# Arsham-001/tsu-emulator

Hardware: AMD Instinct MI355X
Metric: spin-updates/sec on L×L 2D Ising Gibbs sweep; achieved HBM GB/s vs peak (higher is better)
Workload: dtype int8

## Files before the change

### tsu-emulator_amd/csrc/ising2d_tiled.hip

```cpp
#include "ising2d.h"

#include <type_traits>
#include <vector>

typedef short v2s __attribute__((ext_vector_type(2)));
typedef unsigned short v2us __attribute__((ext_vector_type(2)));

struct TiledParams {
    const int8_t* src;
    int8_t* dst;
    long long pitch;
    int rows, nchunks;
    int cols;
    int q_shift;
    int tile_h;
    int flex_ty;
    int r_begin, r_end;
    long long row0, total_rows;
    int wrap_rows, ghost;
    int k;
    int tiles_x;
    int ty_first, ty_stride;
    uint32_t k0, k1, sweep0, tag_hi, tag_lo;
    uint32_t tblH0, tblH1, tblL0, tblL1;
// ... 38 lines not shown

struct PhiloxKeys {
    uint32_t a[10], b[10];
};

static __device__ __forceinline__ PhiloxKeys make_keys(uint32_t k0, uint32_t k1) {
    PhiloxKeys K;
#pragma unroll
    for (int r = 0; r < 10; ++r) {
        uint32_t x = k0 + (uint32_t)r * TSU_PHILOX_W0, y = k1 + (uint32_t)r * TSU_PHILOX_W1;
        asm volatile("v_mov_b32 %0, %1" : "=v"(x) : "s"(x));
        asm volatile("v_mov_b32 %0, %1" : "=v"(y) : "s"(y));
        K.a[r] = x;
        K.b[r] = y;
    }
    return K;
}

static __device__ __forceinline__ u32x4 philox_vk(uint32_t c0, uint32_t c1, uint32_t c2, uint32_t c3, const PhiloxKeys& K) {
#pragma unroll
    for (int r = 0; r < 10; ++r) {
        uint64_t p0 = (uint64_t)TSU_PHILOX_M0 * c0;
        uint64_t p1 = (uint64_t)TSU_PHILOX_M1 * c2;
        uint32_t n0 = tsu_xor3((uint32_t)(p1 >> 32), c1, K.a[r]);
        uint32_t n2 = tsu_xor3((uint32_t)(p0 >> 32), c3, K.b[r]);
        c1 = (uint32_t)p1;
        c3 = (uint32_t)p0;
        c0 = n0;
        c2 = n2;
    }
    return u32x4{c0, c1, c2, c3};
}

struct Rows2Ctx {
    const void* Ps;
    void* Pd;
    const uint64_t* s_thr;
    int tr_lo, npairs;
    int rgf;
    int total_rows;
    int rg_tile0, wrap_tr;
    uint32_t hs, tag_hi, tag_lo, k0, k1;
    uint32_t tblH0, tblH1, tblL0, tblL1;
    uint32_t t3H0, t3H1, t3L0, t3L1;
    int last_row;
    bool lft, rgt;
    uint32_t r_par, r_slot;
    uint32_t rm_lo, rm_hi;
    uint64_t vm_e, vm_o;
    int sh_next, sh_prev;
};

static __device__ __forceinline__ u32x4 compare_octet(const u32x4& w, uint32_t cnt_lo, uint32_t cnt_hi, uint32_t tH0,
                                                      uint32_t tH1, uint32_t tL0, uint32_t tL1) {
    const uint32_t Hl = perm(tH1, tH0, cnt_lo), Ll = perm(tL1, tL0, cnt_lo);
    const uint32_t Hh = perm(tH1, tH0, cnt_hi), Lh = perm(tL1, tL0, cnt_hi);
    u32x4 d;
    d.x = subsat16(w.x, perm(Hl, Ll, 0x05010400u));
    d.y = subsat16(w.y, perm(Hl, Ll, 0x07030602u));
    d.z = subsat16(w.z, perm(Hh, Lh, 0x05010400u));
    d.w = subsat16(w.w, perm(Hh, Lh, 0x07030602u));
    return d;
}

static __device__ __forceinline__ u32x4 compare_octet_open(const u32x4& w, uint32_t cnt_lo, uint32_t cnt_hi, const Rows2Ctx& c,
                                                           bool row_edge, bool l0, bool r7) {
    uint32_t Hl = perm(c.tblH1, c.tblH0, cnt_lo), Ll = perm(c.tblL1, c.tblL0, cnt_lo);
    uint32_t Hh = perm(c.tblH1, c.tblH0, cnt_hi), Lh = perm(c.tblL1, c.tblL0, cnt_hi);
    if (row_edge | l0 | r7) {
        const uint32_t rl = r7 ? c.rm_lo : 0u, rh = r7 ? c.rm_hi : 0u;
        const uint32_t il = cnt_lo + ((row_edge && l0) ? 0x00000004u : 0u) + (row_edge ? (rl & 0x04040404u) : 0u);
        const uint32_t ih = cnt_hi + (row_edge ? (rh & 0x04040404u) : 0u);
        const uint32_t ml = row_edge ? 0xFFFFFFFFu : ((l0 ? 0x000000FFu : 0u) | rl), mh = row_edge ? 0xFFFFFFFFu : rh;
        Hl = (Hl & ~ml) | (perm(c.t3H1, c.t3H0, il) & ml);
        Ll = (Ll & ~ml) | (perm(c.t3L1, c.t3L0, il) & ml);
        Hh = (Hh & ~mh) | (perm(c.t3H1, c.t3H0, ih) & mh);
        Lh = (Lh & ~mh) | (perm(c.t3L1, c.t3L0, ih) & mh);
    }
    u32x4 d;
    d.x = subsat16(w.x, perm(Hl, Ll, 0x05010400u));
    d.y = subsat16(w.y, perm(Hl, Ll, 0x07030602u));
    d.z = subsat16(w.z, perm(Hh, Lh, 0x05010400u));
    d.w = subsat16(w.w, perm(Hh, Lh, 0x07030602u));
    return d;
}

static __device__ __forceinline__ bool has_zero_field(const u32x4& d) {
    const uint32_t mn = minu16(minu16(d.x, d.y), minu16(d.z, d.w));
    return ((mn & 0xFFFFu) == 0) | ((mn >> 16) == 0);
}

static __device__ __forceinline__ uint64_t pack_flags(const u32x4& d) {
    const uint32_t nlo = perm(d.y, d.x, 0x0B0A0908u) & 0x01010101u;
    const uint32_t nhi = perm(d.w, d.z, 0x0B0A0908u) & 0x01010101u;
    return (uint64_t)nlo | ((uint64_t)nhi << 32);
}

template <int NO>
static __device__ __forceinline__ void edge_rows(const Rows2Ctx& c, int to_wrap, int tr, int& rga, int& rgb) {
    constexpr int SPAN = 2 * ((NO - 1 + 63) / NO) + 1;
    const int s_off = to_wrap > 0 ? c.rg_tile0 : c.rg_tile0 - c.total_rows;
    rga = tr + s_off;
    rgb = rga + 1;
    if (__builtin_expect((uint32_t)(to_wrap - 1) < (uint32_t)SPAN, 0)) {
        rga = tr + c.rg_tile0;
        asm volatile("" : "+v"(rga));
        rgb = rga + 1;
        if (rga >= c.total_rows) rga -= c.total_rows;
        if (rgb >= c.total_rows) rgb -= c.total_rows;
    }
}

template <int NO, int P0, bool EDGE, bool OPEN, bool SEAM = false>
static __device__ __forceinline__ void sweep_pairs(const Rows2Ctx& c, const PhiloxKeys& K, int tr_first, int tr_end, int step_rows, int oct,
                                                   uint32_t cq) {
    const char* const ps0 = reinterpret_cast<const char*>(c.Ps);
    const int d_off = (int)(reinterpret_cast<const char*>(c.Pd) - ps0);
    const int off_end = tr_end * NO * 8;
    const int off_step = step_rows * NO * 8;
    int off = (tr_first * NO + oct) * 8;
    int rg = EDGE ? tr_first : c.rgf + (tr_first - c.tr_lo);
    int to_wrap = EDGE ? c.wrap_tr - __builtin_amdgcn_readfirstlane(rg) : 0;
#pragma unroll 1
    for (; off < off_end; off += off_step, rg += step_rows, to_wrap -= step_rows) {
        asm volatile("" : "+v"(off), "+v"(rg));
        const char* ps = ps0 + off;
        const uint64_t R0 = *reinterpret_cast<const uint64_t*>(ps - NO * 8), R1 = *reinterpret_cast<const uint64_t*>(ps);
        const uint64_t R2 = *reinterpret_cast<const uint64_t*>(ps + NO * 8), R3 = *reinterpret_cast<const uint64_t*>(ps + 2 * NO * 8);
        const uint32_t A0 = SEAM ? 0u : *reinterpret_cast<const uint32_t*>(ps + (P0 ? 8 : -4));
        const uint32_t A1 = SEAM ? 0u : *reinterpret_cast<const uint32_t*>(ps + NO * 8 + (P0 ? -4 : 8));
        const uint64_t Na = SEAM ? *reinterpret_cast<const uint64_t*>(ps + (P0 ? 8 : -8)) : 0ull;
        const uint64_t Nb = SEAM ? *reinterpret_cast<const uint64_t*>(ps + NO * 8 + (P0 ? -8 : 8)) : 0ull;
        __builtin_amdgcn_sched_barrier(0);
        int rga = rg, rgb = rg + 1;
        if (EDGE) edge_rows<NO>(c, to_wrap, rg, rga, rgb);
        const u32x4 w0 = philox_vk(cq, (uint32_t)rga, c.hs, c.tag_hi, K);
        const u32x4 w1 = philox_vk(cq, (uint32_t)rgb, c.hs, c.tag_hi, K);
        __builtin_amdgcn_sched_barrier(0);
        const uint32_t C0l = (uint32_t)R1, C0h = (uint32_t)(R1 >> 32), C1l = (uint32_t)R2, C1h = (uint32_t)(R2 >> 32);
        uint32_t S0l = P0 ? __builtin_amdgcn_alignbyte(C0h, C0l, 1) : __builtin_amdgcn_alignbyte(C0l, A0, 3);
        uint32_t S0h = P0 ? __builtin_amdgcn_alignbyte(A0, C0h, 1) : __builtin_amdgcn_alignbyte(C0h, C0l, 3);
        uint32_t S1l = P0 ? __builtin_amdgcn_alignbyte(C1l, A1, 3) : __builtin_amdgcn_alignbyte(C1h, C1l, 1);
        uint32_t S1h = P0 ? __builtin_amdgcn_alignbyte(C1h, C1l, 3) : __builtin_amdgcn_alignbyte(A1, C1h, 1);
        if (SEAM) {
            const uint64_t nxa = (Na & 0xFFull) << c.sh_next, pva = (Na >> c.sh_prev) & 0xFFull;
            const uint64_t nxb = (Nb & 0xFFull) << c.sh_next, pvb = (Nb >> c.sh_prev) & 0xFFull;
            const uint64_t Sa = P0 ? ((R1 >> 8) | nxa) : ((R1 << 8) | pva);
            const uint64_t Sb = P0 ? ((R2 << 8) | pvb) : ((R2 >> 8) | nxb);
            S0l = (uint32_t)Sa; S0h = (uint32_t)(Sa >> 32);
            S1l = (uint32_t)Sb; S1h = (uint32_t)(Sb >> 32);
        }
        const uint32_t ml = C0l + C1l, mh = C0h + C1h;
        const uint32_t cnt0l = (uint32_t)R0 + ml + S0l, cnt0h = (uint32_t)(R0 >> 32) + mh + S0h;
        const uint32_t cnt1l = (uint32_t)R3 + ml + S1l, cnt1h = (uint32_t)(R3 >> 32) + mh + S1h;
        u32x4 d0, d1;
        uint32_t edge_a = 0, edge_b = 0;
        if (OPEN) {
            const bool ea = rga == 0 || rga == c.last_row, eb = rgb == 0 || rgb == c.last_row;
            const bool la = !P0 && c.lft, ra = c.rgt && c.r_par == (uint32_t)P0, lb = P0 && c.lft, rb = c.rgt && c.r_par != (uint32_t)P0;
            d0 = compare_octet_open(w0, cnt0l, cnt0h, c, ea, la, ra);
            d1 = compare_octet_open(w1, cnt1l, cnt1h, c, eb, lb, rb);
            edge_a = (ea ? 1u : 0u) | (la ? 2u : 0u) | (ra ? 4u : 0u) | (c.r_slot << 4);
            edge_b = (eb ? 1u : 0u) | (lb ? 2u : 0u) | (rb ? 4u : 0u) | (c.r_slot << 4);
        } else {
            d0 = compare_octet(w0, cnt0l, cnt0h, c.tblH0, c.tblH1, c.tblL0, c.tblL1);
            d1 = compare_octet(w1, cnt1l, cnt1h, c.tblH0, c.tblH1, c.tblL0, c.tblL1);
        }
        const uint32_t mn = minu16(minu16(minu16(d0.x, d0.y), minu16(d0.z, d0.w)), minu16(minu16(d1.x, d1.y), minu16(d1.z, d1.w)));
        if (__builtin_expect(((mn & 0xFFFFu) == 0) | ((mn >> 16) == 0), 0)) {
            if (has_zero_field(d0)) d0 = resolve_ties(d0, w0, cnt0l, cnt0h, c.s_thr, cq, (uint32_t)rga, c.hs, c.tag_lo, c.k0, c.k1, edge_a);
            if (has_zero_field(d1)) d1 = resolve_ties(d1, w1, cnt1l, cnt1h, c.s_thr, cq, (uint32_t)rgb, c.hs, c.tag_lo, c.k0, c.k1, edge_b);
        }
        char* pd = const_cast<char*>(ps) + d_off;
        uint64_t n0 = pack_flags(d0), n1 = pack_flags(d1);
        if (OPEN) {
            n0 = (rga < 0 || rga > c.last_row) ? 0 : (n0 & (P0 ? c.vm_o : c.vm_e));
            n1 = (rgb < 0 || rgb > c.last_row) ? 0 : (n1 & (P0 ? c.vm_e : c.vm_o));
        }
        if (SEAM) {
            n0 &= c.vm_e;
            n1 &= c.vm_e;
        }
        *reinterpret_cast<uint64_t*>(pd) = n0;
        *reinterpret_cast<uint64_t*>(pd + NO * 8) = n1;
    }
}


static __device__ __forceinline__ uint32_t nib_shift_next(uint32_t X, uint32_t N) {
    const uint32_t hi = (N << 4) | __builtin_amdgcn_ubfe(X, 4u, 4u);
    return __builtin_amdgcn_alignbit(hi, X, 8);
}
static __device__ __forceinline__ uint32_t nib_shift_prev(uint32_t X, uint32_t M) {
    const uint32_t w = ((X << 4) & 0x10000000u) | (M >> 4);
    return __builtin_amdgcn_alignbit(X, w, 24);
}
static __device__ __forceinline__ uint32_t nib_shift_next_seam(uint32_t X, uint32_t N, int pos) {
    return nib_shift_next(X, 0u) | ((N & 0xFu) << pos);
}
static __device__ __forceinline__ uint32_t nib_shift_prev_seam(uint32_t X, uint32_t M, int pos) {
    const uint32_t w = ((X << 4) & 0x10000000u) | (((M >> pos) & 0xFu) << 24);
    return __builtin_amdgcn_alignbit(X, w, 24);
}
static __device__ __forceinline__ uint32_t nib_pack(const u32x4& d) {
    const uint64_t f = pack_flags(d);
    return (uint32_t)f | ((uint32_t)(f >> 32) << 4);
}

template <int NO, int P0, bool EDGE, bool OPEN = false, bool SEAM = false>
static __device__ __forceinline__ void sweep_pairs_nib(const Rows2Ctx& c, const PhiloxKeys& K, int tr_first, int tr_end, int step_rows, int oct,
                                                       uint32_t cq) {
    const char* const ps0 = reinterpret_cast<const char*>(c.Ps);
    const int d_off = (int)(reinterpret_cast<const char*>(c.Pd) - ps0);
    const int off_end = tr_end * NO * 4;
    const int off_step = step_rows * NO * 4;
    int off = (tr_first * NO + oct) * 4;
    int rg = EDGE ? tr_first : c.rgf + (tr_first - c.tr_lo);
    int to_wrap = EDGE ? c.wrap_tr - __builtin_amdgcn_readfirstlane(rg) : 0;
#pragma unroll 1
    for (; off < off_end; off += off_step, rg += step_rows, to_wrap -= step_rows) {
        asm volatile("" : "+v"(off), "+v"(rg));
        const char* ps = ps0 + off;
        const uint32_t R0 = *reinterpret_cast<const uint32_t*>(ps - NO * 4), R1 = *reinterpret_cast<const uint32_t*>(ps);
        const uint32_t R2 = *reinterpret_cast<const uint32_t*>(ps + NO * 4), R3 = *reinterpret_cast<const uint32_t*>(ps + 2 * NO * 4);
        const uint32_t A0 = *reinterpret_cast<const uint32_t*>(ps + (P0 ? 4 : -4));
        const uint32_t A1 = *reinterpret_cast<const uint32_t*>(ps + NO * 4 + (P0 ? -4 : 4));
        __builtin_amdgcn_sched_barrier(0);
        int rga = rg, rgb = rg + 1;
        if (EDGE) edge_rows<NO>(c, to_wrap, rg, rga, rgb);
        const u32x4 w0 = philox_vk(cq, (uint32_t)rga, c.hs, c.tag_hi, K);
        const u32x4 w1 = philox_vk(cq, (uint32_t)rgb, c.hs, c.tag_hi, K);
        __builtin_amdgcn_sched_barrier(0);
        const uint32_t Sa = SEAM ? (P0 ? nib_shift_next_seam(R1, A0, c.sh_next) : nib_shift_prev_seam(R1, A0, c.sh_prev))
                                 : (P0 ? nib_shift_next(R1, A0) : nib_shift_prev(R1, A0));
        const uint32_t Sb = SEAM ? (P0 ? nib_shift_prev_seam(R2, A1, c.sh_prev) : nib_shift_next_seam(R2, A1, c.sh_next))
                                 : (P0 ? nib_shift_prev(R2, A1) : nib_shift_next(R2, A1));
        const uint32_t mid = R1 + R2;
        const uint32_t cnt0 = R0 + mid + Sa, cnt1 = R3 + mid + Sb;
        const uint32_t cnt0l = cnt0 & 0x0F0F0F0Fu, cnt0h = (cnt0 >> 4) & 0x0F0F0F0Fu;
        const uint32_t cnt1l = cnt1 & 0x0F0F0F0Fu, cnt1h = (cnt1 >> 4) & 0x0F0F0F0Fu;
        u32x4 d0, d1;
        uint32_t edge_a = 0, edge_b = 0;
        if (OPEN) {
            const bool ea = rga == 0 || rga == c.last_row, eb = rgb == 0 || rgb == c.last_row;
            const bool la = !P0 && c.lft, ra = c.rgt && c.r_par == (uint32_t)P0, lb = P0 && c.lft, rb = c.rgt && c.r_par != (uint32_t)P0;
            d0 = compare_octet_open(w0, cnt0l, cnt0h, c, ea, la, ra);
            d1 = compare_octet_open(w1, cnt1l, cnt1h, c, eb, lb, rb);
            edge_a = (ea ? 1u : 0u) | (la ? 2u : 0u) | (ra ? 4u : 0u) | (c.r_slot << 4);
            edge_b = (eb ? 1u : 0u) | (lb ? 2u : 0u) | (rb ? 4u : 0u) | (c.r_slot << 4);
        } else {
            d0 = compare_octet(w0, cnt0l, cnt0h, c.tblH0, c.tblH1, c.tblL0, c.tblL1);
            d1 = compare_octet(w1, cnt1l, cnt1h, c.tblH0, c.tblH1, c.tblL0, c.tblL1);
        }
        const uint32_t mn = minu16(minu16(minu16(d0.x, d0.y), minu16(d0.z, d0.w)), minu16(minu16(d1.x, d1.y), minu16(d1.z, d1.w)));
        if (__builtin_expect(((mn & 0xFFFFu) == 0) | ((mn >> 16) == 0), 0)) {
            if (has_zero_field(d0)) d0 = resolve_ties(d0, w0, cnt0l, cnt0h, c.s_thr, cq, (uint32_t)rga, c.hs, c.tag_lo, c.k0, c.k1, edge_a);
            if (has_zero_field(d1)) d1 = resolve_ties(d1, w1, cnt1l, cnt1h, c.s_thr, cq, (uint32_t)rgb, c.hs, c.tag_lo, c.k0, c.k1, edge_b);
        }
        char* pd = const_cast<char*>(ps) + d_off;
        uint32_t n0 = nib_pack(d0), n1 = nib_pack(d1);
        if (OPEN) {
            const uint64_t ma = P0 ? c.vm_o : c.vm_e, mb = P0 ? c.vm_e : c.vm_o;
            n0 = (rga < 0 || rga > c.last_row) ? 0u : (n0 & ((uint32_t)ma | ((uint32_t)(ma >> 32) << 4)));
            n1 = (rgb < 0 || rgb > c.last_row) ? 0u : (n1 & ((uint32_t)mb | ((uint32_t)(mb >> 32) << 4)));
        }
        if (SEAM) {
            const uint32_t m = (uint32_t)c.vm_e | ((uint32_t)(c.vm_e >> 32) << 4);
            n0 &= m;
            n1 &= m;
        }
        *reinterpret_cast<uint32_t*>(pd) = n0;
        *reinterpret_cast<uint32_t*>(pd + NO * 4) = n1;
    }
}

static __device__ __forceinline__ void xst(uint64_t* p, uint64_t v) { __hip_atomic_store(p, v, __ATOMIC_RELAXED, __HIP_MEMORY_SCOPE_AGENT); }
static __device__ __forceinline__ uint64_t xld(const uint64_t* p) { return __hip_atomic_load(p, __ATOMIC_RELAXED, __HIP_MEMORY_SCOPE_AGENT); }

struct ResidentParams {
    uint64_t* xbuf;
    uint32_t gen0;
    int* err;
    int n_gen, k_last, tiles_y;
    int wrap_y;
    int wrap_x;
    long long* dbg;
};

template <int HT, int WO, int THREADS, bool OPEN = false, bool RESIDENT = false, bool NIB = false>
static __device__ __forceinline__ void tile_body(const TiledParams& p, const int8_t* __restrict__ src, int8_t* __restrict__ dst,
                                                 const int k, const uint32_t sweep0, const int tx, const int ty, uint64_t* lds,
                                                 const PhiloxKeys& K, const ResidentParams* R = nullptr) {
    constexpr int NO = WO + 2;
    constexpr int RLMAX = THREADS / NO;
    int H = p.tile_h, row_off = ty * p.tile_h;
    if (p.flex_ty > 0) {
        const long long half = (p.r_end - p.r_begin + 1) / 2;
        row_off = 2 * (int)(ty * half / p.flex_ty);
        H = 2 * (int)((ty + 1) * half / p.flex_ty) - row_off;
    }
    const int TR = H + 4 * k;
    constexpr int RL = RLMAX;
    using E = typename std::conditional<NIB, uint32_t, uint64_t>::type;
    E* plane0 = reinterpret_cast<E*>(lds + 1);
    E* plane1 = plane0 + TR * NO;
    uint64_t* s_thr = reinterpret_cast<uint64_t*>((reinterpret_cast<uintptr_t>(plane1 + TR * NO + NO + 1) + 7u) & ~(uintptr_t)7u);
    const int tid = threadIdx.x;
    if (tid < 25) s_thr[tid] = p.thr[tid];

    const int q0 = tx * WO + p.q_shift, r0 = p.r_begin + row_off, Rb = r0 - 2 * k;

    const int al = tid / NO, oct = tid - al * NO;
    int cqi = q0 - 1 + oct;
    const bool col_out = OPEN && (cqi < 0 || cqi >= p.nchunks);
    if (!OPEN) {
        if (cqi < 0) cqi += p.nchunks;
        if (cqi >= p.nchunks) cqi -= p.nchunks;
        if (cqi >= p.nchunks) cqi -= p.nchunks;
    }
    const uint32_t cq = (uint32_t)cqi;
    int nv = p.cols - 16 * cqi;
    if (col_out) nv = 0;
    if (nv > 16) nv = 16;
    auto first_sites = [](int n) { return n >= 8 ? 0x0101010101010101ull : (((1ull << (8 * n)) - 1) & 0x0101010101010101ull); };
    const uint64_t vm_e = first_sites((nv + 1) >> 1), vm_o = first_sites(nv >> 1);

    if (al < RLMAX) {
        const int8_t* col = src + 16 * (long long)(OPEN ? (cqi < 0 ? 0 : (cqi >= p.nchunks ? p.nchunks - 1 : cqi)) : cqi);
        constexpr int LB = 4;
        for (int tr0 = al; tr0 < TR; tr0 += LB * RLMAX) {
            uint4 v[LB];
#pragma unroll
            for (int b = 0; b < LB; ++b) {
                const int tr = tr0 + b * RLMAX;
                const int rl = Rb + (tr < TR ? tr : TR - 1);
                int srow;
                if (p.wrap_rows) srow = rl < 0 ? rl + p.rows : (rl >= p.rows ? rl - p.rows : rl);
                else srow = rl < -p.ghost ? -p.ghost : (rl >= p.rows + p.ghost ? p.rows + p.ghost - 1 : rl);
                v[b] = *reinterpret_cast<const uint4*>(col + (long long)srow * p.pitch);
            }
#pragma unroll
            for (int b = 0; b < LB; ++b) {
                const int tr = tr0 + b * RLMAX;
                if (tr < TR) {
                    const uint32_t e0 = perm(v[b].y, v[b].x, 0x06040200u), e1 = perm(v[b].w, v[b].z, 0x06040200u);
                    const uint32_t o0 = perm(v[b].y, v[b].x, 0x07050301u), o1 = perm(v[b].w, v[b].z, 0x07050301u);
                    uint64_t ev = (uint64_t)(~(e0 >> 1) & 0x01010101u) | ((uint64_t)(~(e1 >> 1) & 0x01010101u) << 32);
                    uint64_t od = (uint64_t)(~(o0 >> 1) & 0x01010101u) | ((uint64_t)(~(o1 >> 1) & 0x01010101u) << 32);
                    if (OPEN) {
                        const long long grow = p.row0 + Rb + tr;
                        if (grow < 0 || grow >= p.total_rows) ev = od = 0;
                    }
                    if (OPEN || nv < 16) {
                        ev &= vm_e;
                        od &= vm_o;
                    }
                    const int idx = tr * NO + oct;
                    const int gpar = (int)((p.row0 + Rb + tr) & 1);
                    if (NIB) {
                        (gpar ? plane1 : plane0)[idx] = (E)((uint32_t)ev | ((uint32_t)(ev >> 32) << 4));
                        (gpar ? plane0 : plane1)[idx] = (E)((uint32_t)od | ((uint32_t)(od >> 32) << 4));
                    } else {
                        (gpar ? plane1 : plane0)[idx] = (E)ev;
                        (gpar ? plane0 : plane1)[idx] = (E)od;
                    }
                }
            }
        }
    }

    long long rg0 = p.row0 + Rb;
    if (!OPEN) {
        rg0 %= p.total_rows;
        if (rg0 < 0) rg0 += p.total_rows;
    }
    const bool edge = !OPEN && (rg0 + TR > p.total_rows);

    Rows2Ctx c;
    c.s_thr = s_thr;
    c.total_rows = (int)p.total_rows;
    c.rg_tile0 = (int)rg0;
    c.wrap_tr = (int)(p.total_rows - rg0);
    c.tag_hi = p.tag_hi; c.tag_lo = p.tag_lo; c.k0 = p.k0; c.k1 = p.k1;
    c.tblH0 = p.tblH0; c.tblH1 = p.tblH1; c.tblL0 = p.tblL0; c.tblL1 = p.tblL1;
    c.t3H0 = p.t3H0; c.t3H1 = p.t3H1; c.t3L0 = p.t3L0; c.t3L1 = p.t3L1;
    c.last_row = (int)p.total_rows - 1;
    c.lft = OPEN && cqi == 0;
    c.rgt = OPEN && cqi == p.nchunks - 1;
    c.r_par = (uint32_t)(p.cols - 1) & 1u;
    c.r_slot = ((uint32_t)(p.cols - 1) & 15u) >> 1;
    c.rm_lo = c.r_slot < 4 ? 0xFFu << (8 * c.r_slot) : 0u;
    c.rm_hi = c.r_slot < 4 ? 0u : 0xFFu << (8 * (c.r_slot - 4));
    c.vm_e = vm_e;
    c.vm_o = vm_o;
    const int v_last = (p.cols >> 1) & 7;
    const bool ragged = !OPEN && v_last != 0;
    const int seam_site = v_last - 1;
    const int seam_pos = NIB ? 8 * (seam_site & 3) + 4 * (seam_site >> 2) : 8 * seam_site, last_pos = NIB ? 28 : 56;
    c.sh_next = (ragged && cqi == p.nchunks - 1) ? seam_pos : last_pos;
    c.sh_prev = (ragged && cqi == 0) ? seam_pos : last_pos;
    int w0 = (q0 - 1) % p.nchunks;
    if (w0 < 0) w0 += p.nchunks;
    const bool seam = ragged && (w0 == 0 || w0 + NO - 1 >= p.nchunks - 1);
    asm volatile("v_mov_b32 %0, %1" : "=v"(c.tblH0) : "s"(p.tblH0));
    asm volatile("v_mov_b32 %0, %1" : "=v"(c.tblH1) : "s"(p.tblH1));
    asm volatile("v_mov_b32 %0, %1" : "=v"(c.tblL0) : "s"(p.tblL0));
    asm volatile("v_mov_b32 %0, %1" : "=v"(c.tblL1) : "s"(p.tblL1));

    const int n_gen = RESIDENT ? R->n_gen : 1;
    long long tl0 = 0, tl[4] = {0, 0, 0, 0};
    const bool timing = RESIDENT && R->dbg && tid == 0;
    if (timing) tl0 = wall_clock64();
#define RES_MARK(q)                         \
    if (timing) {                           \
        const long long now_ = wall_clock64(); \
// ... 16 lines not shown
        const int ntiles = p.tiles_x * R->tiles_y, me = ty * p.tiles_x + tx;
        uint64_t* mine = R->xbuf + ((size_t)(gen & 1) * ntiles + me) * xstride;
        const uint64_t tag = strip_tag(gen);
        for (int i = tid; i < n_tb; i += THREADS) {
            const int r = i / WO, o = i - r * WO;
            xst(mine + i, (uint64_t)plane1[(2 * k + r) * NO + 1 + o] | tag);
            xst(mine + n_tb + i, (uint64_t)plane1[(H + r) * NO + 1 + o] | tag);
        }
        for (int i = tid; i < n_lr; i += THREADS) {
            xst(mine + 2 * n_tb + i, (uint64_t)plane1[(2 * k + i) * NO + 1] | tag);
            xst(mine + 2 * n_tb + n_lr + i, (uint64_t)plane1[(2 * k + i) * NO + wi] | tag);
        }
        RES_MARK(1);
    };
    auto fetch = [&](int gen) {
        RES_MARK(0);
        const int tiles_x = p.tiles_x, tiles_y = R->tiles_y, ntiles = tiles_x * tiles_y;
        const uint64_t tag = strip_tag(gen);
        const int txl = tx == 0 ? tiles_x - 1 : tx - 1, txr = tx == tiles_x - 1 ? 0 : tx + 1;
        const int w_l = txl == tiles_x - 1 ? p.nchunks + p.q_shift - (txl * WO + p.q_shift) : WO;
        const int tyu = ty == 0 ? tiles_y - 1 : ty - 1, tyd = ty == tiles_y - 1 ? 0 : ty + 1;
        const bool has_u = R->wrap_y || ty > 0, has_d = R->wrap_y || ty < tiles_y - 1;
        const bool has_l = R->wrap_x || tx > 0, has_r = R->wrap_x || tx < tiles_x - 1;
        const uint64_t* xg = R->xbuf + (size_t)(gen & 1) * ntiles * xstride;
        const uint64_t* X_u = xg + (size_t)(tyu * tiles_x + tx) * xstride;
        const uint64_t* X_d = xg + (size_t)(tyd * tiles_x + tx) * xstride;
        const uint64_t* X_l = xg + (size_t)(ty * tiles_x + txl) * xstride;
        const uint64_t* X_r = xg + (size_t)(ty * tiles_x + txr) * xstride;
        const uint64_t* X_ul = xg + (size_t)(tyu * tiles_x + txl) * xstride;
        const uint64_t* X_ur = xg + (size_t)(tyu * tiles_x + txr) * xstride;
        const uint64_t* X_dl = xg + (size_t)(tyd * tiles_x + txl) * xstride;
        const uint64_t* X_dr = xg + (size_t)(tyd * tiles_x + txr) * xstride;
        constexpr int FI = (2 * 8 * NO + THREADS - 1) / THREADS;
        constexpr int TH_MAX = 160 * 1024 / (int)sizeof(E) / (2 * NO) - 32;
        constexpr int SI = (TH_MAX + THREADS - 1) / THREADS;
        const uint64_t* au[FI];
        const uint64_t* ad[FI];
        uint64_t vu[FI], vd[FI], vl[SI], vr[SI];
        bool nu[FI], nd[FI], nl[SI], nr[SI];
#pragma unroll
        for (int it = 0; it < FI; ++it) {
            const int i = tid + it * THREADS, ic = i < 2 * k * NO ? i : 0;
            const int r = ic / NO, o = ic - r * NO;
            const int e = r * WO;
            const int oc = o <= wi + 1 ? o : 1;
            au[it] = oc == 0 ? X_ul + n_tb + e + w_l - 1 : (oc == wi + 1 ? X_ur + n_tb + e : X_u + n_tb + e + oc - 1);
            ad[it] = oc == 0 ? X_dl + e + w_l - 1 : (oc == wi + 1 ? X_dr + e : X_d + e + oc - 1);
            const bool col_ok = o == 0 ? has_l : (o == wi + 1 ? has_r : o <= wi);
            nu[it] = i < 2 * k * NO && has_u && col_ok;
            nd[it] = i < 2 * k * NO && has_d && col_ok;
            vu[it] = xld(au[it]);
            vd[it] = xld(ad[it]);
        }
#pragma unroll
        for (int it = 0; it < SI; ++it) {
            const int i = tid + it * THREADS, ic = i < n_lr ? i : 0;
            nl[it] = i < n_lr && has_l;
            nr[it] = i < n_lr && has_r;
            vl[it] = xld(X_l + 2 * n_tb + n_lr + ic);
            vr[it] = xld(X_r + 2 * n_tb + ic);
        }
        for (int spins = 0;; ++spins) {
            bool fresh = true;
#pragma unroll
            for (int it = 0; it < FI; ++it) {
                if (nu[it] && (vu[it] & TAG_MASK) != tag) { vu[it] = xld(au[it]); fresh = false; }
                if (nd[it] && (vd[it] & TAG_MASK) != tag) { vd[it] = xld(ad[it]); fresh = false; }
// ... 4 lines not shown
                if (nl[it] && (vl[it] & TAG_MASK) != tag) { vl[it] = xld(X_l + 2 * n_tb + n_lr + ic); fresh = false; }
                if (nr[it] && (vr[it] & TAG_MASK) != tag) { vr[it] = xld(X_r + 2 * n_tb + ic); fresh = false; }
            }
            if (fresh) break;
            if (spins > (1 << 22) || ((spins & 0xFFF) == 0xFFF && __hip_atomic_load(R->err, __ATOMIC_RELAXED, __HIP_MEMORY_SCOPE_SYSTEM))) {
                __hip_atomic_store(R->err, 1, __ATOMIC_RELAXED, __HIP_MEMORY_SCOPE_SYSTEM);
                s_fail = 1;
                break;
            }
        }
        RES_MARK(2);
#pragma unroll
        for (int it = 0; it < FI; ++it) {
            const int i = tid + it * THREADS;
            if (i < 2 * k * NO) {
                const int r = i / NO, o = i - r * NO;
                if (nu[it]) plane1[r * NO + o] = (E)(vu[it] & FLAG_MASK);
                if (nd[it]) plane1[(2 * k + H + r) * NO + o] = (E)(vd[it] & FLAG_MASK);
            }
        }
#pragma unroll
        for (int it = 0; it < SI; ++it) {
            const int i = tid + it * THREADS;
            if (i < n_lr) {
                if (nl[it]) plane1[(2 * k + i) * NO] = (E)(vl[it] & FLAG_MASK);
                if (nr[it]) plane1[(2 * k + i) * NO + wi + 1] = (E)(vr[it] & FLAG_MASK);
            }
        }
        RES_MARK(3);
    };

    auto run = [&](int par0, int tr_first, int tr_end, int step, int oc, uint32_t cqq) {
        if (NIB && OPEN) {
            if (par0) sweep_pairs_nib<NO, 1, false, true>(c, K, tr_first, tr_end, step, oc, cqq);
            else sweep_pairs_nib<NO, 0, false, true>(c, K, tr_first, tr_end, step, oc, cqq);
        } else if (NIB && seam) {
            if (par0) sweep_pairs_nib<NO, 1, true, false, true>(c, K, tr_first, tr_end, step, oc, cqq);
            else sweep_pairs_nib<NO, 0, true, false, true>(c, K, tr_first, tr_end, step, oc, cqq);
        } else if (NIB) {
            if (edge) {
                if (par0) sweep_pairs_nib<NO, 1, true>(c, K, tr_first, tr_end, step, oc, cqq);
                else sweep_pairs_nib<NO, 0, true>(c, K, tr_first, tr_end, step, oc, cqq);
            } else {
                if (par0) sweep_pairs_nib<NO, 1, false>(c, K, tr_first, tr_end, step, oc, cqq);
                else sweep_pairs_nib<NO, 0, false>(c, K, tr_first, tr_end, step, oc, cqq);
            }
        } else if (OPEN) {
            if (par0) sweep_pairs<NO, 1, false, true>(c, K, tr_first, tr_end, step, oc, cqq);
            else sweep_pairs<NO, 0, false, true>(c, K, tr_first, tr_end, step, oc, cqq);
        } else if (seam) {
            if (par0) sweep_pairs<NO, 1, true, false, true>(c, K, tr_first, tr_end, step, oc, cqq);
            else sweep_pairs<NO, 0, true, false, true>(c, K, tr_first, tr_end, step, oc, cqq);
        } else if (edge) {
            if (par0) sweep_pairs<NO, 1, true, false>(c, K, tr_first, tr_end, step, oc, cqq);
            else sweep_pairs<NO, 0, true, false>(c, K, tr_first, tr_end, step, oc, cqq);
        } else {
            if (par0) sweep_pairs<NO, 1, false, false>(c, K, tr_first, tr_end, step, oc, cqq);
            else sweep_pairs<NO, 0, false, false>(c, K, tr_first, tr_end, step, oc, cqq);
        }
    };
    int par0 = 0;
    auto set_half_sweep = [&](uint32_t sweep_g, int hsi) {
        const int kappa = hsi & 1;
        c.hs = 2u * (sweep_g + (uint32_t)(hsi >> 1)) + (uint32_t)kappa;
        c.Pd = kappa ? plane1 : plane0;
        c.Ps = kappa ? plane0 : plane1;
        c.tr_lo = 1 + hsi;
        c.npairs = (TR - 2 - 2 * hsi) / 2;
        int rgf = (int)rg0 + c.tr_lo;
        if (!OPEN && rgf >= c.total_rows) rgf -= c.total_rows;
        c.rgf = rgf;
        par0 = (int)((p.row0 + Rb + c.tr_lo + kappa) & 1);
    };
    for (int gen = 0; gen < n_gen; ++gen) {
    const int kg = (RESIDENT && gen == n_gen - 1) ? R->k_last : k;
    const uint32_t sweep_g = sweep0 + (uint32_t)(gen * k);
    for (int hsi = 0; hsi < 2 * kg; ++hsi) {
        __syncthreads();
        set_half_sweep(sweep_g, hsi);
        if (al < RL) run(par0, c.tr_lo + 2 * al, c.tr_lo + 2 * c.npairs, 2 * RL, oct, cq);
    }
    __syncthreads();
    if (RESIDENT && gen + 1 < n_gen) {
        publish(gen);
        fetch(gen);
        __syncthreads();
        if (s_fail) return;
    }
    RES_MARK(0);
    }
    if (timing)
        for (int q = 0; q < 4; ++q) R->dbg[4 * blockIdx.x + q] = tl[q];
#undef RES_MARK
    if (al < RLMAX && oct >= 1 && oct <= WO && q0 + oct - 1 < p.nchunks + p.q_shift) {
        int8_t* col = dst + 16 * (long long)cqi;
        int gpar = (int)((p.row0 + r0 + al) & 1);
#pragma unroll 2
        for (int hr = al; hr < H; hr += RLMAX) {
            const int rl = r0 + hr;
            if (rl < p.r_end) {
                const int li = (2 * k + hr) * NO + oct;
                uint64_t ev = (gpar ? plane1 : plane0)[li], od = (gpar ? plane0 : plane1)[li];
                if (NIB) {
                    ev = (ev & 0x01010101ull) | (((ev >> 4) & 0x01010101ull) << 32);
                    od = (od & 0x01010101ull) | (((od >> 4) & 0x01010101ull) << 32);
                }
                const uint32_t e0 = perm(0u, 0x000001FFu, (uint32_t)ev), e1 = perm(0u, 0x000001FFu, (uint32_t)(ev >> 32));
                const uint32_t o0 = perm(0u, 0x000001FFu, (uint32_t)od), o1 = perm(0u, 0x000001FFu, (uint32_t)(od >> 32));
                uint4 v = make_uint4(perm(o0, e0, 0x05010400u), perm(o0, e0, 0x07030602u), perm(o1, e1, 0x05010400u),
                                     perm(o1, e1, 0x07030602u));
// ... 15 lines not shown
__global__ __launch_bounds__(THREADS, MINW) void k1_tiled2(TiledParams p) {
    extern __shared__ uint64_t lds[];
    const PhiloxKeys K = make_keys(p.k0, p.k1);
    tile_body<H, WO, THREADS, OPEN, false, NIB>(p, p.src, p.dst, p.k, p.sweep0, blockIdx.x % p.tiles_x,
                                    p.ty_first + (blockIdx.x / p.tiles_x) * p.ty_stride, lds, K);
}

struct ResidentLaunch {
    TiledParams t;
    ResidentParams r;
};

template <int H, int WO, int THREADS, int MINW = 1, bool OPEN = false, bool NIB = false>
__global__ __launch_bounds__(THREADS, MINW) void k1_resident(ResidentLaunch P) {
    extern __shared__ uint64_t lds[];
    const PhiloxKeys K = make_keys(P.t.k0, P.t.k1);
    tile_body<H, WO, THREADS, OPEN, true, NIB>(P.t, P.t.src, P.t.dst, P.t.k, P.t.sweep0, blockIdx.x % P.t.tiles_x, blockIdx.x / P.t.tiles_x,
                                          lds, K, &P.r);
}

namespace {
constexpr int KMAX = 8;

struct TileVariant {
    int H, WO, threads;
    void (*kernel)(TiledParams);
    void (*resident)(ResidentLaunch);
    void (*open)(TiledParams);
    void (*resident_open)(ResidentLaunch);
    int nib;
    int per_cu;
};

size_t tile_lds_bytes(const TileVariant& tv, int TR) {
    const size_t es = tv.nib ? 4 : 8, NO = (size_t)tv.WO + 2;
    return 8 + (((size_t)2 * TR * NO + NO + 1) * es + 7) / 8 * 8 + 8 + 25 * sizeof(uint64_t);
}
enum { V_64x512_T512 = 0, V_128x512_T512, V_128x512_T1024, V_256x512_T1024, V_128x256_T1024, V_64x512_T1024, V_64x256_T1024, V_32x256_T1024,
       V_N512x512_T1024, V_N256x512_T512 };
const TileVariant kVariants[] = {
    {64, 32, 512, k1_tiled2<64, 32, 512>, k1_resident<64, 32, 512>, k1_tiled2<64, 32, 512, 1, true>, nullptr, 0, 2},
    {128, 32, 512, k1_tiled2<128, 32, 512>, k1_resident<128, 32, 512>, k1_tiled2<128, 32, 512, 1, true>, nullptr, 0, 2},
    {128, 32, 1024, k1_tiled2<128, 32, 1024>, k1_resident<128, 32, 1024>, k1_tiled2<128, 32, 1024, 1, true>, k1_resident<128, 32, 1024, 1, true>, 0, 1},
    {256, 32, 1024, k1_tiled2<256, 32, 1024, 4>, k1_resident<256, 32, 1024, 4>, k1_tiled2<256, 32, 1024, 4, true>, k1_resident<256, 32, 1024, 4, true>, 0, 1},
    {128, 16, 1024, k1_tiled2<128, 16, 1024>, k1_resident<128, 16, 1024>, k1_tiled2<128, 16, 1024, 1, true>, k1_resident<128, 16, 1024, 1, true>, 0, 1},
    {64, 32, 1024, k1_tiled2<64, 32, 1024>, k1_resident<64, 32, 1024>, k1_tiled2<64, 32, 1024, 1, true>, k1_resident<64, 32, 1024, 1, true>, 0, 1},
    {64, 16, 1024, k1_tiled2<64, 16, 1024>, k1_resident<64, 16, 1024>, k1_tiled2<64, 16, 1024, 1, true>, k1_resident<64, 16, 1024, 1, true>, 0, 1},
    {32, 16, 1024, k1_tiled2<32, 16, 1024>, k1_resident<32, 16, 1024>, k1_tiled2<32, 16, 1024, 1, true>, k1_resident<32, 16, 1024, 1, true>, 0, 1},
    {512, 32, 1024, k1_tiled2<512, 32, 1024, 4, false, true>, k1_resident<512, 32, 1024, 4, false, true>, k1_tiled2<512, 32, 1024, 4, true, true>,
     k1_resident<512, 32, 1024, 4, true, true>, 1, 1},
    {256, 32, 512, k1_tiled2<256, 32, 512, 4, false, true>, nullptr, k1_tiled2<256, 32, 512, 4, true, true>, nullptr, 1, 2},
};
constexpr int kNumVariants = sizeof(kVariants) / sizeof(kVariants[0]);

int ragged_shift(const tsu_ising2d* L, int WO) {
    if (!L->periodic || L->cols % 16 == 0) return 0;
    const int nch = (L->cols + 15) / 16, tiles_x = (nch + WO - 1) / WO;
    for (int shift = 1; shift < WO && shift < nch - 1; ++shift) {
        bool ok = true;
        for (int t = 0; t < tiles_x && ok; ++t) {
            const int s = t * WO + shift;
            if (s % nch == 0) ok = false;
            if (t < tiles_x - 1 && (s + WO) % nch == nch - 1) ok = false;
        }
        if (ok) return shift;
    }
    return -1;
}

size_t lds_share(const TileVariant& tv) { return (size_t)(160 / tv.per_cu) * 1024; }
// ... 563 lines not shown
```

Before: 3014 billion.

## Precompute Philox first rounds per row and column; table row products in LDS

Splits the Philox counter-based RNG into column-invariant, row-invariant and per-row parts. The first rounds depend only on (column chunk, tag, keys) or on (row, half-sweep), so they are computed once per thread or once per row and kept in LDS. Each inner-loop Philox then starts from a partially advanced state. The per-row global row index is now tabulated in LDS, which removes the wraparound edge_rows branch and the separate edge kernel instantiations. The cost is more LDS per tile (which lowers the maximum tile height) and extra LDS loads in the hot loop.

```diff
diff --git a/tsu-emulator_amd/csrc/ising2d_tiled.hip b/tsu-emulator_amd/csrc/ising2d_tiled.hip
--- a/tsu-emulator_amd/csrc/ising2d_tiled.hip
+++ b/tsu-emulator_amd/csrc/ising2d_tiled.hip
@@ -94,14 +94,67 @@
     return u32x4{c0, c1, c2, c3};
 }
 
+static __device__ __forceinline__ uint64_t row_product(uint32_t row, uint32_t hs, uint32_t k0) {
+    return (uint64_t)TSU_PHILOX_M0 * ((uint32_t)(((uint64_t)TSU_PHILOX_M1 * hs) >> 32) ^ row ^ k0);
+}
+
+static constexpr __host__ __device__ bool row_products_fit(int threads) { return threads >= 1024; }
+
+template <bool ETAB>
+using lds_rowp = const __attribute__((address_space(3))) typename std::conditional<ETAB, uint64_t, uint32_t>::type*;
+
+struct ColInv {
+    uint32_t qa1, x1, x2;
+};
+struct RowInv {
+    uint32_t x1, x2, x3, c3b3;
+};
+
+static __device__ __forceinline__ ColInv make_col_inv(uint32_t cq, uint32_t tag, uint32_t k0, uint32_t k1) {
+    const uint64_t p0 = (uint64_t)TSU_PHILOX_M0 * cq;
+    const uint64_t Q = (uint64_t)TSU_PHILOX_M1 * ((uint32_t)(p0 >> 32) ^ tag ^ k1);
+    return ColInv{(uint32_t)(Q >> 32) ^ (k0 + TSU_PHILOX_W0), (uint32_t)p0 ^ (k1 + TSU_PHILOX_W1), (uint32_t)Q ^ (k0 + 2u * TSU_PHILOX_W0)};
+}
+static __device__ __forceinline__ RowInv make_row_inv(const ColInv& ci, uint32_t hs, uint32_t k1) {
+    const uint64_t F = (uint64_t)TSU_PHILOX_M0 * (ci.qa1 ^ (uint32_t)((uint64_t)TSU_PHILOX_M1 * hs));
+    RowInv v{ci.x1, ci.x2, (uint32_t)(F >> 32) ^ (k1 + 2u * TSU_PHILOX_W1), (uint32_t)F ^ (k1 + 3u * TSU_PHILOX_W1)};
+    asm volatile("" : "+v"(v.x3), "+v"(v.c3b3));
+    return v;
+}
+
+static __device__ __forceinline__ u32x4 philox_from_row(uint64_t E, const RowInv& v, const PhiloxKeys& K) {
+    const uint64_t P = (uint64_t)TSU_PHILOX_M1 * ((uint32_t)(E >> 32) ^ v.x1);
+    uint32_t c0 = (uint32_t)(P >> 32) ^ v.x2, c1 = (uint32_t)P, c2 = (uint32_t)E ^ v.x3, c3;
+    {
+        const uint64_t p0 = (uint64_t)TSU_PHILOX_M0 * c0, p1 = (uint64_t)TSU_PHILOX_M1 * c2;
+        c0 = tsu_xor3((uint32_t)(p1 >> 32), c1, K.a[3]);
+        c2 = (uint32_t)(p0 >> 32) ^ v.c3b3;
+        c1 = (uint32_t)p1;
+        c3 = (uint32_t)p0;
+    }
+#pragma unroll
+    for (int r = 4; r < 10; ++r) {
+        const uint64_t p0 = (uint64_t)TSU_PHILOX_M0 * c0, p1 = (uint64_t)TSU_PHILOX_M1 * c2;
+        const uint32_t n0 = tsu_xor3((uint32_t)(p1 >> 32), c1, K.a[r]);
+        const uint32_t n2 = tsu_xor3((uint32_t)(p0 >> 32), c3, K.b[r]);
+        c1 = (uint32_t)p1;
+        c3 = (uint32_t)p0;
+        c0 = n0;
+        c2 = n2;
+    }
+    return u32x4{c0, c1, c2, c3};
+}
+
 struct Rows2Ctx {
     const void* Ps;
     void* Pd;
     const uint64_t* s_thr;
+    const uint64_t* Erow;
+    uint32_t urow;
+    const uint32_t* s_row;
+    RowInv inv;
     int tr_lo, npairs;
     int rgf;
-    int total_rows;
-    int rg_tile0, wrap_tr;
     uint32_t hs, tag_hi, tag_lo, k0, k1;
     uint32_t tblH0, tblH1, tblL0, tblL1;
     uint32_t t3H0, t3H1, t3L0, t3L1;
@@ -158,22 +211,7 @@
     return (uint64_t)nlo | ((uint64_t)nhi << 32);
 }
 
-template <int NO>
-static __device__ __forceinline__ void edge_rows(const Rows2Ctx& c, int to_wrap, int tr, int& rga, int& rgb) {
-    constexpr int SPAN = 2 * ((NO - 1 + 63) / NO) + 1;
-    const int s_off = to_wrap > 0 ? c.rg_tile0 : c.rg_tile0 - c.total_rows;
-    rga = tr + s_off;
-    rgb = rga + 1;
-    if (__builtin_expect((uint32_t)(to_wrap - 1) < (uint32_t)SPAN, 0)) {
-        rga = tr + c.rg_tile0;
-        asm volatile("" : "+v"(rga));
-        rgb = rga + 1;
-        if (rga >= c.total_rows) rga -= c.total_rows;
-        if (rgb >= c.total_rows) rgb -= c.total_rows;
-    }
-}
-
-template <int NO, int P0, bool EDGE, bool OPEN, bool SEAM = false>
+template <int NO, int P0, bool ETAB, bool OPEN, bool SEAM = false>
 static __device__ __forceinline__ void sweep_pairs(const Rows2Ctx& c, const PhiloxKeys& K, int tr_first, int tr_end, int step_rows, int oct,
                                                    uint32_t cq) {
     const char* const ps0 = reinterpret_cast<const char*>(c.Ps);
@@ -181,11 +219,19 @@
     const int off_end = tr_end * NO * 8;
     const int off_step = step_rows * NO * 8;
     int off = (tr_first * NO + oct) * 8;
-    int rg = EDGE ? tr_first : c.rgf + (tr_first - c.tr_lo);
-    int to_wrap = EDGE ? c.wrap_tr - __builtin_amdgcn_readfirstlane(rg) : 0;
+    const lds_rowp<ETAB> pe0 = ETAB ? (lds_rowp<ETAB>)c.Erow : (lds_rowp<ETAB>)c.s_row;
+    lds_rowp<ETAB> pe = pe0 + tr_first;
+    int rg = OPEN ? c.rgf + (tr_first - c.tr_lo) : 0;
+    const lds_rowp<ETAB> pe_rg0 = pe0 + (c.tr_lo - c.rgf);
 #pragma unroll 1
-    for (; off < off_end; off += off_step, rg += step_rows, to_wrap -= step_rows) {
-        asm volatile("" : "+v"(off), "+v"(rg));
+    for (; off < off_end; off += off_step, pe += OPEN ? 0 : step_rows, rg += OPEN ? step_rows : 0) {
+        asm volatile("" : "+v"(off));
+        if (OPEN) {
+            asm volatile("" : "+v"(rg));
+            pe = pe_rg0 + rg;
+        } else {
+            asm volatile("" : "+v"(pe));
+        }
         const char* ps = ps0 + off;
         const uint64_t R0 = *reinterpret_cast<const uint64_t*>(ps - NO * 8), R1 = *reinterpret_cast<const uint64_t*>(ps);
         const uint64_t R2 = *reinterpret_cast<const uint64_t*>(ps + NO * 8), R3 = *reinterpret_cast<const uint64_t*>(ps + 2 * NO * 8);
@@ -193,11 +239,12 @@
         const uint32_t A1 = SEAM ? 0u : *reinterpret_cast<const uint32_t*>(ps + NO * 8 + (P0 ? -4 : 8));
         const uint64_t Na = SEAM ? *reinterpret_cast<const uint64_t*>(ps + (P0 ? 8 : -8)) : 0ull;
         const uint64_t Nb = SEAM ? *reinterpret_cast<const uint64_t*>(ps + NO * 8 + (P0 ? -8 : 8)) : 0ull;
+        const uint64_t Ea = ETAB ? (uint64_t)pe[0] : (uint64_t)TSU_PHILOX_M0 * (c.urow ^ (uint32_t)pe[0]);
+        const uint64_t Eb = ETAB ? (uint64_t)pe[1] : (uint64_t)TSU_PHILOX_M0 * (c.urow ^ (uint32_t)pe[1]);
         __builtin_amdgcn_sched_barrier(0);
-        int rga = rg, rgb = rg + 1;
-        if (EDGE) edge_rows<NO>(c, to_wrap, rg, rga, rgb);
-        const u32x4 w0 = philox_vk(cq, (uint32_t)rga, c.hs, c.tag_hi, K);
-        const u32x4 w1 = philox_vk(cq, (uint32_t)rgb, c.hs, c.tag_hi, K);
+        const int rga = rg, rgb = rg + 1;
+        const u32x4 w0 = philox_from_row(Ea, c.inv, K);
+        const u32x4 w1 = philox_from_row(Eb, c.inv, K);
         __builtin_amdgcn_sched_barrier(0);
         const uint32_t C0l = (uint32_t)R1, C0h = (uint32_t)(R1 >> 32), C1l = (uint32_t)R2, C1h = (uint32_t)(R2 >> 32);
         uint32_t S0l = P0 ? __builtin_amdgcn_alignbyte(C0h, C0l, 1) : __builtin_amdgcn_alignbyte(C0l, A0, 3);
@@ -230,8 +277,9 @@
         }
         const uint32_t mn = minu16(minu16(minu16(d0.x, d0.y), minu16(d0.z, d0.w)), minu16(minu16(d1.x, d1.y), minu16(d1.z, d1.w)));
         if (__builtin_expect(((mn & 0xFFFFu) == 0) | ((mn >> 16) == 0), 0)) {
-            if (has_zero_field(d0)) d0 = resolve_ties(d0, w0, cnt0l, cnt0h, c.s_thr, cq, (uint32_t)rga, c.hs, c.tag_lo, c.k0, c.k1, edge_a);
-            if (has_zero_field(d1)) d1 = resolve_ties(d1, w1, cnt1l, cnt1h, c.s_thr, cq, (uint32_t)rgb, c.hs, c.tag_lo, c.k0, c.k1, edge_b);
+            const uint32_t* rw = c.s_row + (pe - pe0);
+            if (has_zero_field(d0)) d0 = resolve_ties(d0, w0, cnt0l, cnt0h, c.s_thr, cq, rw[0], c.hs, c.tag_lo, c.k0, c.k1, edge_a);
+            if (has_zero_field(d1)) d1 = resolve_ties(d1, w1, cnt1l, cnt1h, c.s_thr, cq, rw[1], c.hs, c.tag_lo, c.k0, c.k1, edge_b);
         }
         char* pd = const_cast<char*>(ps) + d_off;
         uint64_t n0 = pack_flags(d0), n1 = pack_flags(d1);
@@ -269,7 +317,7 @@
     return (uint32_t)f | ((uint32_t)(f >> 32) << 4);
 }
 
-template <int NO, int P0, bool EDGE, bool OPEN = false, bool SEAM = false>
+template <int NO, int P0, bool ETAB, bool OPEN = false, bool SEAM = false>
 static __device__ __forceinline__ void sweep_pairs_nib(const Rows2Ctx& c, const PhiloxKeys& K, int tr_first, int tr_end, int step_rows, int oct,
                                                        uint32_t cq) {
     const char* const ps0 = reinterpret_cast<const char*>(c.Ps);
@@ -277,21 +325,30 @@
     const int off_end = tr_end * NO * 4;
     const int off_step = step_rows * NO * 4;
     int off = (tr_first * NO + oct) * 4;
-    int rg = EDGE ? tr_first : c.rgf + (tr_first - c.tr_lo);
-    int to_wrap = EDGE ? c.wrap_tr - __builtin_amdgcn_readfirstlane(rg) : 0;
+    const lds_rowp<ETAB> pe0 = ETAB ? (lds_rowp<ETAB>)c.Erow : (lds_rowp<ETAB>)c.s_row;
+    lds_rowp<ETAB> pe = pe0 + tr_first;
+    int rg = OPEN ? c.rgf + (tr_first - c.tr_lo) : 0;
+    const lds_rowp<ETAB> pe_rg0 = pe0 + (c.tr_lo - c.rgf);
 #pragma unroll 1
-    for (; off < off_end; off += off_step, rg += step_rows, to_wrap -= step_rows) {
-        asm volatile("" : "+v"(off), "+v"(rg));
+    for (; off < off_end; off += off_step, pe += OPEN ? 0 : step_rows, rg += OPEN ? step_rows : 0) {
+        asm volatile("" : "+v"(off));
+        if (OPEN) {
+            asm volatile("" : "+v"(rg));
+            pe = pe_rg0 + rg;
+        } else {
+            asm volatile("" : "+v"(pe));
+        }
         const char* ps = ps0 + off;
         const uint32_t R0 = *reinterpret_cast<const uint32_t*>(ps - NO * 4), R1 = *reinterpret_cast<const uint32_t*>(ps);
         const uint32_t R2 = *reinterpret_cast<const uint32_t*>(ps + NO * 4), R3 = *reinterpret_cast<const uint32_t*>(ps + 2 * NO * 4);
         const uint32_t A0 = *reinterpret_cast<const uint32_t*>(ps + (P0 ? 4 : -4));
         const uint32_t A1 = *reinterpret_cast<const uint32_t*>(ps + NO * 4 + (P0 ? -4 : 4));
+        const uint64_t Ea = ETAB ? (uint64_t)pe[0] : (uint64_t)TSU_PHILOX_M0 * (c.urow ^ (uint32_t)pe[0]);
+        const uint64_t Eb = ETAB ? (uint64_t)pe[1] : (uint64_t)TSU_PHILOX_M0 * (c.urow ^ (uint32_t)pe[1]);
         __builtin_amdgcn_sched_barrier(0);
-        int rga = rg, rgb = rg + 1;
-        if (EDGE) edge_rows<NO>(c, to_wrap, rg, rga, rgb);
-        const u32x4 w0 = philox_vk(cq, (uint32_t)rga, c.hs, c.tag_hi, K);
-        const u32x4 w1 = philox_vk(cq, (uint32_t)rgb, c.hs, c.tag_hi, K);
+        const int rga = rg, rgb = rg + 1;
+        const u32x4 w0 = philox_from_row(Ea, c.inv, K);
+        const u32x4 w1 = philox_from_row(Eb, c.inv, K);
         __builtin_amdgcn_sched_barrier(0);
         const uint32_t Sa = SEAM ? (P0 ? nib_shift_next_seam(R1, A0, c.sh_next) : nib_shift_prev_seam(R1, A0, c.sh_prev))
                                  : (P0 ? nib_shift_next(R1, A0) : nib_shift_prev(R1, A0));
@@ -316,8 +373,9 @@
         }
         const uint32_t mn = minu16(minu16(minu16(d0.x, d0.y), minu16(d0.z, d0.w)), minu16(minu16(d1.x, d1.y), minu16(d1.z, d1.w)));
         if (__builtin_expect(((mn & 0xFFFFu) == 0) | ((mn >> 16) == 0), 0)) {
-            if (has_zero_field(d0)) d0 = resolve_ties(d0, w0, cnt0l, cnt0h, c.s_thr, cq, (uint32_t)rga, c.hs, c.tag_lo, c.k0, c.k1, edge_a);
-            if (has_zero_field(d1)) d1 = resolve_ties(d1, w1, cnt1l, cnt1h, c.s_thr, cq, (uint32_t)rgb, c.hs, c.tag_lo, c.k0, c.k1, edge_b);
+            const uint32_t* rw = c.s_row + (pe - pe0);
+            if (has_zero_field(d0)) d0 = resolve_ties(d0, w0, cnt0l, cnt0h, c.s_thr, cq, rw[0], c.hs, c.tag_lo, c.k0, c.k1, edge_a);
+            if (has_zero_field(d1)) d1 = resolve_ties(d1, w1, cnt1l, cnt1h, c.s_thr, cq, rw[1], c.hs, c.tag_lo, c.k0, c.k1, edge_b);
         }
         char* pd = const_cast<char*>(ps) + d_off;
         uint32_t n0 = nib_pack(d0), n1 = nib_pack(d1);
@@ -348,6 +406,10 @@
     int wrap_x;
     long long* dbg;
 };
+
+static constexpr __host__ __device__ size_t tile_lds_layout(size_t es, size_t NO, size_t TR, bool etab) {
+    return 8 + ((2 * TR * NO + NO + 1) * es + 7) / 8 * 8 + 8 + 25 * 8 + (etab ? 2 * TR * 8 : 0) + (TR * 4 + 7) / 8 * 8;
+}
 
 template <int HT, int WO, int THREADS, bool OPEN = false, bool RESIDENT = false, bool NIB = false>
 static __device__ __forceinline__ void tile_body(const TiledParams& p, const int8_t* __restrict__ src, int8_t* __restrict__ dst,
@@ -366,7 +428,10 @@
     using E = typename std::conditional<NIB, uint32_t, uint64_t>::type;
     E* plane0 = reinterpret_cast<E*>(lds + 1);
     E* plane1 = plane0 + TR * NO;
-    uint64_t* s_thr = reinterpret_cast<uint64_t*>((reinterpret_cast<uintptr_t>(plane1 + TR * NO + NO + 1) + 7u) & ~(uintptr_t)7u);
+    uint64_t* s_thr = lds + 1 + ((size_t)(2 * TR * NO + NO + 1) * sizeof(E) + 7) / 8;
+    constexpr bool ETAB = row_products_fit(THREADS);
+    uint64_t* const s_E = s_thr + 25;
+    uint32_t* const s_row = reinterpret_cast<uint32_t*>(s_E + (ETAB ? 2 * TR : 0));
     const int tid = threadIdx.x;
     if (tid < 25) s_thr[tid] = p.thr[tid];
 
@@ -381,6 +446,7 @@
         if (cqi >= p.nchunks) cqi -= p.nchunks;
     }
     const uint32_t cq = (uint32_t)cqi;
+    const ColInv col_inv = make_col_inv(cq, p.tag_hi, p.k0, p.k1);
     int nv = p.cols - 16 * cqi;
     if (col_out) nv = 0;
     if (nv > 16) nv = 16;
@@ -436,13 +502,19 @@
         rg0 %= p.total_rows;
         if (rg0 < 0) rg0 += p.total_rows;
     }
-    const bool edge = !OPEN && (rg0 + TR > p.total_rows);
+    for (int tr = tid; tr < TR; tr += THREADS) {
+        int rg = (int)rg0 + tr;
+        if (!OPEN && rg >= (int)p.total_rows) rg -= (int)p.total_rows;
+        s_row[tr] = (uint32_t)rg;
+    }
+    auto fill_rows = [&](uint32_t hs, int buf) {
+        if (!ETAB) return;
+        for (int tr = tid; tr < TR; tr += THREADS) s_E[buf * TR + tr] = row_product(s_row[tr], hs, p.k0);
+    };
 
     Rows2Ctx c;
     c.s_thr = s_thr;
-    c.total_rows = (int)p.total_rows;
-    c.rg_tile0 = (int)rg0;
-    c.wrap_tr = (int)(p.total_rows - rg0);
+    c.s_row = s_row;
     c.tag_hi = p.tag_hi; c.tag_lo = p.tag_lo; c.k0 = p.k0; c.k1 = p.k1;
     c.tblH0 = p.tblH0; c.tblH1 = p.tblH1; c.tblL0 = p.tblL0; c.tblL1 = p.tblL1;
     c.t3H0 = p.t3H0; c.t3H1 = p.t3H1; c.t3L0 = p.t3L0; c.t3L1 = p.t3L1;
@@ -525,7 +597,8 @@
         const uint64_t* X_dl = xg + (size_t)(tyd * tiles_x + txl) * xstride;
         const uint64_t* X_dr = xg + (size_t)(tyd * tiles_x + txr) * xstride;
         constexpr int FI = (2 * 8 * NO + THREADS - 1) / THREADS;
-        constexpr int TH_MAX = 160 * 1024 / (int)sizeof(E) / (2 * NO) - 32;
+        constexpr int TH_MAX = (int)((160 * 1024 - tile_lds_layout(sizeof(E), NO, 0, ETAB)) / (2 * NO * sizeof(E) + (ETAB ? 20 : 4))) + 1 - 32;
+        static_assert(tile_lds_layout(sizeof(E), NO, TH_MAX + 32, ETAB) > 160 * 1024, "TH_MAX is no upper bound");
         constexpr int SI = (TH_MAX + THREADS - 1) / THREADS;
         const uint64_t* au[FI];
         const uint64_t* ad[FI];
@@ -596,31 +669,23 @@
 
     auto run = [&](int par0, int tr_first, int tr_end, int step, int oc, uint32_t cqq) {
         if (NIB && OPEN) {
-            if (par0) sweep_pairs_nib<NO, 1, false, true>(c, K, tr_first, tr_end, step, oc, cqq);
-            else sweep_pairs_nib<NO, 0, false, true>(c, K, tr_first, tr_end, step, oc, cqq);
+            if (par0) sweep_pairs_nib<NO, 1, ETAB, true>(c, K, tr_first, tr_end, step, oc, cqq);
+            else sweep_pairs_nib<NO, 0, ETAB, true>(c, K, tr_first, tr_end, step, oc, cqq);
         } else if (NIB && seam) {
-            if (par0) sweep_pairs_nib<NO, 1, true, false, true>(c, K, tr_first, tr_end, step, oc, cqq);
-            else sweep_pairs_nib<NO, 0, true, false, true>(c, K, tr_first, tr_end, step, oc, cqq);
+            if (par0) sweep_pairs_nib<NO, 1, ETAB, false, true>(c, K, tr_first, tr_end, step, oc, cqq);
+            else sweep_pairs_nib<NO, 0, ETAB, false, true>(c, K, tr_first, tr_end, step, oc, cqq);
         } else if (NIB) {
-            if (edge) {
-                if (par0) sweep_pairs_nib<NO, 1, true>(c, K, tr_first, tr_end, step, oc, cqq);
-                else sweep_pairs_nib<NO, 0, true>(c, K, tr_first, tr_end, step, oc, cqq);
-            } else {
-                if (par0) sweep_pairs_nib<NO, 1, false>(c, K, tr_first, tr_end, step, oc, cqq);
-                else sweep_pairs_nib<NO, 0, false>(c, K, tr_first, tr_end, step, oc, cqq);
-            }
+            if (par0) sweep_pairs_nib<NO, 1, ETAB>(c, K, tr_first, tr_end, step, oc, cqq);
+            else sweep_pairs_nib<NO, 0, ETAB>(c, K, tr_first, tr_end, step, oc, cqq);
         } else if (OPEN) {
-            if (par0) sweep_pairs<NO, 1, false, true>(c, K, tr_first, tr_end, step, oc, cqq);
-            else sweep_pairs<NO, 0, false, true>(c, K, tr_first, tr_end, step, oc, cqq);
+            if (par0) sweep_pairs<NO, 1, ETAB, true>(c, K, tr_first, tr_end, step, oc, cqq);
+            else sweep_pairs<NO, 0, ETAB, true>(c, K, tr_first, tr_end, step, oc, cqq);
         } else if (seam) {
-            if (par0) sweep_pairs<NO, 1, true, false, true>(c, K, tr_first, tr_end, step, oc, cqq);
-            else sweep_pairs<NO, 0, true, false, true>(c, K, tr_first, tr_end, step, oc, cqq);
-        } else if (edge) {
-            if (par0) sweep_pairs<NO, 1, true, false>(c, K, tr_first, tr_end, step, oc, cqq);
-            else sweep_pairs<NO, 0, true, false>(c, K, tr_first, tr_end, step, oc, cqq);
+            if (par0) sweep_pairs<NO, 1, ETAB, false, true>(c, K, tr_first, tr_end, step, oc, cqq);
+            else sweep_pairs<NO, 0, ETAB, false, true>(c, K, tr_first, tr_end, step, oc, cqq);
         } else {
-            if (par0) sweep_pairs<NO, 1, false, false>(c, K, tr_first, tr_end, step, oc, cqq);
-            else sweep_pairs<NO, 0, false, false>(c, K, tr_first, tr_end, step, oc, cqq);
+            if (par0) sweep_pairs<NO, 1, ETAB, false>(c, K, tr_first, tr_end, step, oc, cqq);
+            else sweep_pairs<NO, 0, ETAB, false>(c, K, tr_first, tr_end, step, oc, cqq);
         }
     };
     int par0 = 0;
@@ -629,17 +694,19 @@
         c.hs = 2u * (sweep_g + (uint32_t)(hsi >> 1)) + (uint32_t)kappa;
         c.Pd = kappa ? plane1 : plane0;
         c.Ps = kappa ? plane0 : plane1;
+        c.Erow = s_E + kappa * TR;
+        c.urow = (uint32_t)(((uint64_t)TSU_PHILOX_M1 * c.hs) >> 32) ^ p.k0;
+        c.inv = make_row_inv(col_inv, c.hs, p.k1);
         c.tr_lo = 1 + hsi;
         c.npairs = (TR - 2 - 2 * hsi) / 2;
-        int rgf = (int)rg0 + c.tr_lo;
-        if (!OPEN && rgf >= c.total_rows) rgf -= c.total_rows;
-        c.rgf = rgf;
+        c.rgf = (int)rg0 + c.tr_lo;
         par0 = (int)((p.row0 + Rb + c.tr_lo + kappa) & 1);
     };
     for (int gen = 0; gen < n_gen; ++gen) {
     const int kg = (RESIDENT && gen == n_gen - 1) ? R->k_last : k;
     const uint32_t sweep_g = sweep0 + (uint32_t)(gen * k);
     for (int hsi = 0; hsi < 2 * kg; ++hsi) {
+        fill_rows(2u * (sweep_g + (uint32_t)(hsi >> 1)) + (uint32_t)(hsi & 1), hsi & 1);
         __syncthreads();
         set_half_sweep(sweep_g, hsi);
         if (al < RL) run(par0, c.tr_lo + 2 * al, c.tr_lo + 2 * c.npairs, 2 * RL, oct, cq);
@@ -721,10 +788,7 @@
     int per_cu;
 };
 
-size_t tile_lds_bytes(const TileVariant& tv, int TR) {
-    const size_t es = tv.nib ? 4 : 8, NO = (size_t)tv.WO + 2;
-    return 8 + (((size_t)2 * TR * NO + NO + 1) * es + 7) / 8 * 8 + 8 + 25 * sizeof(uint64_t);
-}
+size_t tile_lds_bytes(const TileVariant& tv, int TR) { return tile_lds_layout(tv.nib ? 4 : 8, tv.WO + 2, TR, row_products_fit(tv.threads)); }
 enum { V_64x512_T512 = 0, V_128x512_T512, V_128x512_T1024, V_256x512_T1024, V_128x256_T1024, V_64x512_T1024, V_64x256_T1024, V_32x256_T1024,
        V_N512x512_T1024, V_N256x512_T512 };
 const TileVariant kVariants[] = {
```

Measured after the change: 2908 billion. 3.5% lower.
